# aalto-speech/AaltoASR

Measured on AMD Instinct MI355X. Metric: frames/sec GMM log-lik (39-d, 50k Gauss) + MFCC, 1/2/4/8 MI355X, higher is better.
Workload: dtype f32 (2-term fp16 split on the matrix cores, f32 accumulate); 1 GPU; configs[2]: full MFCC chain (FFT -> mel -> log -> DCT -> delta/delta-delta, CMS, normalisation) + 50000-Gaussian scoring + 2-byte LNA codes on 1 h of synthetic 16 kHz audio as 360 x 10 s utterances (449280 frames), int16 samples resident in HBM; dim=39, gaussians=50000, states=3125, gpus_flag=1

## Files before the change

### aaltoasr_amd/capi.py

```python
from __future__ import annotations

import ctypes as C
import os
import re
from typing import Optional

import numpy as np

HERE = os.path.dirname(os.path.abspath(__file__))
LIB_PATH = os.path.join(os.environ.get("AASR_LIBDIR") or os.path.join(HERE, "lib"), "libaasr.so")
HEADER_PATH = os.path.join(HERE, "..", "include", "aasr.h")

AASR_OK = 0
AASR_ERR_INVALID = -1
AASR_ERR_UNSUPPORTED = -2
AASR_ERR_NO_DEVICE = -3
AASR_ERR_IO = -4
AASR_ERR_SHORT_AUDIO = -5


class AasrError(RuntimeError):
    def __init__(self, code: int, msg: str):
        super().__init__("aasr status %d: %s" % (code, msg))
        self.code = code
# ... 596 lines not shown
        out = np.empty((n_frames, dim), dtype)
        fn = lib().aasr_feat_run if dtype == np.float32 else lib().aasr_feat_run_f64
        check(fn(self._h, _ptr(pcm), len(pcm), first_frame, n_frames,
                 module.encode() if module else None, _ptr(out)))
        return out

    def run_features(self, frames: np.ndarray, first_frame: int, n_frames: int,
                     module: Optional[str] = None, dtype=np.float32) -> np.ndarray:
        frames = np.ascontiguousarray(frames, np.float32)
        dim = self.module_dim(module) if module else self.dim
        out = np.empty((n_frames, dim), dtype)
        fn = lib().aasr_feat_run_features if dtype == np.float32 else lib().aasr_feat_run_features_f64
        check(fn(self._h, _ptr(frames), frames.size, first_frame, n_frames,
                 module.encode() if module else None, _ptr(out)))
        return out

    def run_batch_dev(self, d_pcm, pcm_off: np.ndarray, frame_off: np.ndarray, d_out, stream=None):
        pcm_off = np.ascontiguousarray(pcm_off, np.int64)
        frame_off = np.ascontiguousarray(frame_off, np.int64)
        check(lib().aasr_feat_run_batch_dev(self._h, _ptr(d_pcm), _ptr(pcm_off), _ptr(frame_off),
                                            len(pcm_off) - 1, _ptr(d_out), _stream_handle(stream)))

    def set_parameters(self, module: str, block_text: str) -> None:
        check(lib().aasr_feat_set_parameters(self._h, module.encode(), block_text.encode()))

    def get_parameters(self, module: str) -> str:
        out = C.c_void_p()
        n = C.c_int64()
        check(lib().aasr_feat_get_parameters(self._h, module.encode(), C.byref(out), C.byref(n)))
        try:
            return C.string_at(out, n.value).decode()
        finally:
            lib().aasr_free(out)

    def modules(self):
        L = lib()
        return [(L.aasr_feat_module_name(self._h, i).decode(), L.aasr_feat_module_type(self._h, i).decode())
                for i in range(L.aasr_feat_num_modules(self._h))]


def recipe_batch_range(total: int, num_batches: int, batch_index: int):
    f, n = C.c_int32(), C.c_int32()
    check(lib().aasr_recipe_batch_range(total, num_batches, batch_index, C.byref(f), C.byref(n)))
    return f.value, n.value


def debug_feat_fusion(on: bool) -> None:
    L = lib()
    L.aasr_debug_feat_fusion.argtypes = [C.c_int]
    L.aasr_debug_feat_fusion.restype = None
    L.aasr_debug_feat_fusion(int(on))


def debug_cluster_heap(on: bool) -> None:
    L = lib()
    L.aasr_debug_cluster_heap.argtypes = [C.c_int]
    L.aasr_debug_cluster_heap.restype = None
    L.aasr_debug_cluster_heap(int(on))


def recipe_frame_limits(start_time: float, end_time: float, frame_rate: float):
    a, b = C.c_int32(), C.c_int32()
    lib().aasr_recipe_frame_limits(start_time, end_time, frame_rate, C.byref(a), C.byref(b))
    return a.value, b.value


def recipe_read(text, num_batches: int = 0, batch_index: int = 0):
    out = C.c_void_p()
    n = C.c_int64()
    raw = text if isinstance(text, bytes) else text.encode()
    check(lib().aasr_recipe_read(raw, num_batches, batch_index, C.byref(out), C.byref(n)))
    try:
        table = C.string_at(out, n.value)
    finally:
        lib().aasr_free(out)
    rows = []
    for line in table.split(b"\n")[:-1]:
        f = line.split(b"\x1f")
        rows.append(tuple(x.decode("latin-1") for x in f[:4]) +
                    (float(np.float32(float(f[4]))), float(np.float32(float(f[5])))))
    return rows


def recipe_read_all(text, num_batches: int = 0, batch_index: int = 0, cluster_speakers: bool = False):
    out = C.c_void_p()
    n = C.c_int64()
    raw = text if isinstance(text, bytes) else text.encode()
    check(lib().aasr_recipe_read_all(raw, num_batches, batch_index, int(cluster_speakers), C.byref(out), C.byref(n)))
    try:
        table = C.string_at(out, n.value)
    finally:
        lib().aasr_free(out)
    rows = []
    for line in table.split(b"\n")[:-1]:
        f = [x.decode("latin-1") for x in line.split(b"\x1f")]
        rows.append(tuple(f[:7]) + (float(np.float32(float(f[7]))), float(np.float32(float(f[8]))),
                                    int(f[9]), int(f[10]), f[11], f[12]))
    return rows


def lna_read_file(path: str):
    out = C.POINTER(C.c_float)()
    S = C.c_int32()
    nb = C.c_int32()
    F = C.c_int64()
    check(lib().aasr_lna_read_file(path.encode(), C.byref(S), C.byref(nb), C.byref(F), C.byref(out)))
# ... 548 lines not shown
```

### aaltoasr_amd/csrc/feat_kernels.hip

```cpp
#include <hip/hip_runtime.h>

#include <cmath>
#include <cstring>
#include <climits>

#include "feat.h"

namespace aasr {

struct DevBatch {
  int n_utts;
  const int64_t *frame_off;
  const int64_t *pcm_off;
  const int32_t *first;
  const int32_t *eof_frame;
};

__device__ __forceinline__ int find_utt(const DevBatch &b, int64_t r, int span) {
  int lo = 0, hi = b.n_utts - 1;
  while (lo < hi) {
    int mid = (lo + hi + 1) >> 1;
    int64_t key = b.frame_off[mid] + (int64_t)mid * span;
    if (key <= r) lo = mid; else hi = mid - 1;
  }
// ... 360 lines not shown
#endif
#if AASR_ABLATION
#define AASR_FDBG(bits) (dbg & (bits))
#else
#define AASR_FDBG(bits) false
#endif
constexpr int SPEC_FRAMES = 16;
constexpr int SPEC_TPF = 16;

struct SpectralPrm {
  FftPrm fp;
  int mel_dim, mel_root, mel_terms;
  const int32_t *mel_off, *mel_t, *mel_order;
  const float *mel_scale, *mel_sum;
  int dct_dim, zeroth;
  const float *dct_cos;
};

typedef float spec_tbl_t;
struct SpectralLds {
  size_t bufs, frame_u, melv, powv, ham, perm, tw, stw, moff, mt, msc, msum, mord, dct, prm, total;
  size_t frame_u_stride;
  __host__ __device__ SpectralLds(int nc, int mel_dim, int mel_terms, int dct_rows) {
    size_t o = 0;
    auto take = [&](size_t n) {
      size_t at = o;
      o += (n + 15) & ~(size_t)15;
      return at;
    };
    bufs = take((size_t)SPEC_FRAMES * nc * 8);
    const size_t pcm_b = (size_t)(2 * nc + 2) * 2, spec_b = (size_t)((nc + 1) | 1) * 4;
    frame_u_stride = ((pcm_b > spec_b ? pcm_b : spec_b) + 7) & ~(size_t)7;
    frame_u_stride |= 4;
    frame_u = take((size_t)SPEC_FRAMES * frame_u_stride);
    melv = take((size_t)SPEC_FRAMES * mel_dim * 8);
    powv = 0;
    ham = take((size_t)2 * nc * sizeof(spec_tbl_t));
    perm = take((size_t)nc * 4);
    tw = take((size_t)nc * 8);
    stw = take((size_t)(nc / 2 + 1) * 8);
    moff = take((size_t)(mel_dim + 1) * 4);
    mt = take((size_t)mel_terms * 4);
    msc = take((size_t)mel_terms * sizeof(spec_tbl_t));
    msum = take((size_t)mel_dim * 4);
    mord = take((size_t)mel_dim * 4);
    dct = take((size_t)dct_rows * mel_dim * sizeof(spec_tbl_t));
    prm = take((size_t)SPEC_FRAMES * 3 * 8);
    total = o;
  }
};

__global__ __launch_bounds__(256) void k_spectral_fused(DevBatch b, const int16_t *__restrict__ pcm,
                                                        AudioPrm ap, int L, int R, int64_t rows,
                                                        SpectralPrm sp, int passes, int dbg,
                                                        double *__restrict__ dst) {
  extern __shared__ __attribute__((aligned(16))) char smem_raw[];
  constexpr int FB = SPEC_FRAMES, TPF = SPEC_TPF;
  const int nc = sp.fp.nc, nbins = nc + 1;
  const int dct_rows = sp.dct_dim - (sp.zeroth ? 1 : 0);
  const SpectralLds lds(nc, sp.mel_dim, sp.mel_terms, dct_rows);
  cpx *bufs = (cpx *)(smem_raw + lds.bufs);
  double *melv = (double *)(smem_raw + lds.melv);
  spec_tbl_t *t_ham = (spec_tbl_t *)(smem_raw + lds.ham);
  int32_t *t_perm = (int32_t *)(smem_raw + lds.perm);
  cpx *t_tw = (cpx *)(smem_raw + lds.tw);
  cpx *t_stw = (cpx *)(smem_raw + lds.stw);
  int32_t *t_moff = (int32_t *)(smem_raw + lds.moff);
  int32_t *t_mt = (int32_t *)(smem_raw + lds.mt);
  spec_tbl_t *t_msc = (spec_tbl_t *)(smem_raw + lds.msc);
  float *t_msum = (float *)(smem_raw + lds.msum);
  int32_t *t_mord = (int32_t *)(smem_raw + lds.mord);
  spec_tbl_t *t_dct = (spec_tbl_t *)(smem_raw + lds.dct);
  int64_t *s_prm = (int64_t *)(smem_raw + lds.prm);
  const int tid = threadIdx.x;
  const int f = tid / TPF, l = tid - f * TPF;

  for (int i = tid; i < 2 * nc; i += 256) t_ham[i] = (spec_tbl_t)sp.fp.hamming[i];
  for (int i = tid; i < nc; i += 256) {
    t_perm[i] = sp.fp.perm[i];
    t_tw[i] = ((const cpx *)sp.fp.twiddle)[i];
  }
  for (int i = tid; i < nc / 2; i += 256) t_stw[i] = ((const cpx *)sp.fp.stwiddle)[i];
  for (int i = tid; i <= sp.mel_dim; i += 256) t_moff[i] = sp.mel_off[i];
  for (int i = tid; i < sp.mel_terms; i += 256) {
    t_mt[i] = sp.mel_t[i];
    t_msc[i] = (spec_tbl_t)sp.mel_scale[i];
  }
  for (int i = tid; i < sp.mel_dim; i += 256) {
    t_msum[i] = sp.mel_sum[i];
    t_mord[i] = sp.mel_order[i];
  }
  for (int i = tid; i < dct_rows * sp.mel_dim; i += 256) t_dct[i] = (spec_tbl_t)sp.dct_cos[i];

  cpx *buf = bufs + (size_t)f * nc;
  char *fu = smem_raw + lds.frame_u + (size_t)f * lds.frame_u_stride;
  float *spec = (float *)fu;
  const int out_dim = sp.dct_dim + 1;
  const int64_t nblk = (rows + FB - 1) / FB;
  int u_cur = -1;
  for (int pass = 0; pass < passes; pass++) {
    const int64_t blk = (int64_t)blockIdx.x * passes + pass;
    if (blk >= nblk) break;
    const int64_t r0 = blk * FB;
    __syncthreads();
    if (tid < FB) {
      int64_t r = r0 + tid;
      if (r > rows - 1) r = rows - 1;
      int u;
      if (AASR_FDBG(1)) {
        u = 0;
      } else if (u_cur < 0) {
        u = find_utt_near(b, r, L + R, rows);
      } else {
        u = u_cur;
        while (u + 1 < b.n_utts && b.frame_off[u + 1] + (int64_t)(u + 1) * (L + R) <= r) u++;
      }
      u_cur = u;
      const int frame = b.first[u] - L + (int)(r - (b.frame_off[u] + (int64_t)u * (L + R)));
      s_prm[3 * tid] = window_start(b, u, frame, ap);
      s_prm[3 * tid + 1] = b.pcm_off[u];
      s_prm[3 * tid + 2] = b.pcm_off[u + 1] - b.pcm_off[u];
    }
    __syncthreads();
    {
      const int64_t ws = s_prm[3 * f], ns = s_prm[3 * f + 2];
      const int16_t *p = pcm + s_prm[3 * f + 1];
      const bool inside = ws >= 0 && ws + 2 * nc < ns;
      auto point = [&](int o) {
        const int s = t_perm[o];
        float c0, c1, c2;
        if (inside) {
          const int16_t *q = p + ws + 2 * s;
          c0 = (float)q[0];
          c1 = (float)q[1];
          c2 = (float)q[2];
        } else {
          const int64_t i = ws + 2 * s;
          c0 = (i >= 0 && i < ns) ? (float)p[i] : 0.0f;
          c1 = (i + 1 >= 0 && i + 1 < ns) ? (float)p[i + 1] : 0.0f;
          c2 = (i + 2 >= 0 && i + 2 < ns) ? (float)p[i + 2] : 0.0f;
        }
        const float p0 = ap.emph * c0, p1 = ap.emph * c1;
        cpx v;
        v.r = t_ham[2 * s] * (c1 - p0);
        v.i = t_ham[2 * s + 1] * (c2 - p1);
        return v;
      };
      for (int o = l; o < ((AASR_FDBG(32) || AASR_FDBG(8)) ? 0 : nc); o += TPF) buf[o] = point(o);
    }
    __builtin_amdgcn_fence(__ATOMIC_RELEASE, "wavefront");
    __builtin_amdgcn_wave_barrier();
    for (int st = AASR_FDBG(2) ? -1 : sp.fp.ns - 1; st >= 0; st--) {
      const int pr = sp.fp.radix[st], m = sp.fp.sublen[st];
      const int fstride = sp.fp.fstride[st];
      const int nb = fstride * m;
      for (int bi = l; bi < nb; bi += TPF) kiss_butterfly(buf, bi, pr, m, sp.fp.sub_magic[st], fstride, t_tw);
      __builtin_amdgcn_fence(__ATOMIC_RELEASE, "wavefront");
      __builtin_amdgcn_wave_barrier();
    }
    if (l == 0 && !AASR_FDBG(64)) {
      const cpx t0 = buf[0];
      spec[0] = spec_value(t0.r + t0.i, 0.0f, sp.fp.magnitude, sp.fp.take_log);
      spec[nc] = spec_value(t0.r - t0.i, 0.0f, sp.fp.magnitude, sp.fp.take_log);
    }
    for (int k0 = l; k0 < (AASR_FDBG(64) ? 0 : nc / 2); k0 += TPF) {
      const int k = k0 == 0 ? nc / 2 : k0;
      float re_k, im_k, re_n, im_n;
      real_split(buf, nc, k, t_stw, re_k, im_k, re_n, im_n);
      if (k != nc - k) spec[k] = spec_value(re_k, im_k, sp.fp.magnitude, sp.fp.take_log);
      spec[nc - k] = spec_value(re_n, im_n, sp.fp.magnitude, sp.fp.take_log);
// ... 48 lines not shown
    __builtin_amdgcn_fence(__ATOMIC_RELEASE, "wavefront");
    __builtin_amdgcn_wave_barrier();
    if (r0 + f < rows && !AASR_FDBG(128)) {
      const double *data = melv + (size_t)f * sp.mel_dim;
      for (int i = l; i < sp.dct_dim; i += TPF) {
        double acc = 0.0;
        if (sp.zeroth && i == 0) {
          for (int k = 0; k < sp.mel_dim; k++) acc += data[k];
        } else {
          const spec_tbl_t *c = t_dct + (size_t)(i - (sp.zeroth ? 1 : 0)) * sp.mel_dim;
#pragma unroll 4
          for (int k = 0; k < sp.mel_dim; k++) acc += data[k] * (double)c[k];
        }
        dst[(r0 + f) * out_dim + i] = acc;
      }
    }
    __builtin_amdgcn_fence(__ATOMIC_RELEASE, "wavefront");
    __builtin_amdgcn_wave_barrier();
  }
}

struct TemporalPrm {
  int dx, w1, w2;
  float norm1, norm2;
  const float *mean, *scale;
  const float *matrix, *bias;
  int dim;
};

#ifdef AASR_TR
constexpr int kTemporalRows = AASR_TR;
#else
constexpr int kTemporalRows = 64;
#endif

static inline size_t temporal_smem(int tile_rows, int dx, int H, int w2, int dim) {
  return (size_t)(tile_rows + 2 * H) * dx * 8 + (size_t)(tile_rows + 2 * w2) * dx * 8 + (size_t)tile_rows * 3 * dx * 8 + 16 +
         (size_t)(3 * dx) * ((dim + 2) / 3) * 16 + (size_t)(6 * dx + dim) * 4;
}

template <int ROWS, int NT>
__global__ __launch_bounds__(NT) void k_temporal_fused(DevBatch b, const double *__restrict__ src,
                                                        SrcMap sm, int span, int64_t rows,
                                                        TemporalPrm tp, int dbg, double *__restrict__ dst) {
  extern __shared__ __attribute__((aligned(16))) char smem_raw[];
  const int dx = tp.dx, H = tp.w1 + tp.w2, md = 3 * tp.dx;
  const unsigned dx_magic = fast_magic(dx), dim_magic = fast_magic(tp.dim);
  double *xs = (double *)smem_raw;
  double *d1 = xs + (size_t)(ROWS + 2 * H) * dx;
  double *nrm = d1 + (size_t)(ROWS + 2 * tp.w2) * dx;
  float4 *mt = (float4 *)(smem_raw + ((((size_t)(2 * ROWS + 2 * H + 2 * tp.w2) * dx + (size_t)ROWS * md) * 8 + 15) & ~(size_t)15));
  const int ngrp = (tp.dim + 2) / 3;
  const unsigned ngrp_magic = fast_magic(ngrp);
  if (tp.matrix && !AASR_FDBG(8))
    for (int e = threadIdx.x; e < md * ngrp; e += NT) {
      const int j = fast_div(e, ngrp_magic), g = e - j * ngrp;
      float4 v;
      v.x = tp.matrix[(size_t)(3 * g) * md + j];
      v.y = 3 * g + 1 < tp.dim ? tp.matrix[(size_t)(3 * g + 1) * md + j] : 0.0f;
      v.z = 3 * g + 2 < tp.dim ? tp.matrix[(size_t)(3 * g + 2) * md + j] : 0.0f;
      v.w = 0.0f;
      mt[e] = v;
    }
  float *nmean = (float *)(mt + (size_t)md * ngrp), *nscale = nmean + md, *nbias = nscale + md;
  for (int e = threadIdx.x; e < md; e += NT) {
    nmean[e] = tp.mean[e];
    nscale[e] = tp.scale[e];
  }
  if (tp.bias)
    for (int e = threadIdx.x; e < tp.dim; e += NT) nbias[e] = tp.bias[e];
  const int64_t tile0 = (int64_t)blockIdx.x * ROWS;
  const int64_t tile1 = tile0 + ROWS < rows ? tile0 + ROWS : rows;
  int64_t r0 = tile0;
  while (r0 < tile1) {
    const int u = AASR_FDBG(64) ? 0 : find_utt_near(b, r0, span, rows);
    const int64_t u_end = AASR_FDBG(64) ? rows : b.frame_off[u + 1] + (int64_t)(u + 1) * span;
    const int64_t r_end = u_end < tile1 ? u_end : tile1;
    const int64_t s0 = r0 + (int64_t)u * sm.span_diff + sm.shift;
    const int n_seg = (int)(r_end - r0);
    const int n_x = n_seg + 2 * H, n_d1 = n_seg + 2 * tp.w2;
    for (int e = threadIdx.x; e < (AASR_FDBG(16) ? 0 : n_x * dx); e += NT) xs[e] = src[(s0 - H) * dx + e];
    __syncthreads();
    for (int e = threadIdx.x; e < (AASR_FDBG(4) ? 0 : n_d1 * dx); e += NT) {
      const int j = fast_div(e, dx_magic), i = e - j * dx;
      const int c = j + tp.w1;
      double acc = 0;
      for (int k = 1; k <= tp.w1; k++) {
        const double left = xs[(size_t)(c - k) * dx + i];
        const double right = xs[(size_t)(c + k) * dx + i];
        acc += k * (right - left);
      }
      d1[e] = acc / (double)tp.norm1;
    }
    __syncthreads();
    for (int e = threadIdx.x; e < (AASR_FDBG(2) ? 0 : n_seg * dx); e += NT) {
      const int lr = fast_div(e, dx_magic), i = e - lr * dx;
      const double v0 = xs[(size_t)(lr + H) * dx + i];
      const double v1 = d1[(size_t)(lr + tp.w2) * dx + i];
      const int c = lr + tp.w2;
      double acc = 0;
      for (int k = 1; k <= tp.w2; k++) {
        const double left = d1[(size_t)(c - k) * dx + i];
        const double right = d1[(size_t)(c + k) * dx + i];
        acc += k * (right - left);
      }
      const double v2 = acc / (double)tp.norm2;
      double *o = nrm + (size_t)lr * md + i;
      o[0] = (v0 - (double)nmean[i]) * (double)nscale[i];
      o[dx] = (v1 - (double)nmean[dx + i]) * (double)nscale[dx + i];
      o[2 * dx] = (v2 - (double)nmean[2 * dx + i]) * (double)nscale[2 * dx + i];
    }
    __syncthreads();
    if (tp.matrix) {
      const int npair = (n_seg + 1) / 2;
      for (int it = threadIdx.x; it < ngrp * npair; it += NT) {
        const int rp = fast_div(it, ngrp_magic), g = it - rp * ngrp;
        const int la = 2 * rp, lb = 2 * rp + 1 < n_seg ? 2 * rp + 1 : la;
        const double *xa = nrm + (size_t)la * md, *xb = nrm + (size_t)lb * md;
        const float4 *mg = mt + g;
        double a0 = 0, a1 = 0, a2 = 0, b0 = 0, b1 = 0, b2 = 0;
        if (!AASR_FDBG(1)) {
#pragma unroll 3
          for (int j = 0; j < md; j++) {
            const float4 m = mg[j * ngrp];
            const double va = xa[j], vb = xb[j];
            const double m0 = (double)m.x, m1 = (double)m.y, m2 = (double)m.z;
            a0 += m0 * va;
            a1 += m1 * va;
            a2 += m2 * va;
            b0 += m0 * vb;
            b1 += m1 * vb;
            b2 += m2 * vb;
          }
        }
        const int i0 = 3 * g;
        if (tp.bias) {
          const double c0 = (double)nbias[i0];
          const double c1 = i0 + 1 < tp.dim ? (double)nbias[i0 + 1] : 0.0;
          const double c2 = i0 + 2 < tp.dim ? (double)nbias[i0 + 2] : 0.0;
          a0 += c0;
          b0 += c0;
          a1 += c1;
          b1 += c1;
          a2 += c2;
          b2 += c2;
        }
        if (AASR_FDBG(32) && a0 != 12345.0) continue;
        double *da = dst + (r0 + la) * tp.dim + i0;
        da[0] = a0;
        if (i0 + 1 < tp.dim) da[1] = a1;
        if (i0 + 2 < tp.dim) da[2] = a2;
        if (lb != la) {
          double *db = dst + (r0 + lb) * tp.dim + i0;
          db[0] = b0;
          if (i0 + 1 < tp.dim) db[1] = b1;
          if (i0 + 2 < tp.dim) db[2] = b2;
        }
      }
    } else {
      for (int e = threadIdx.x; e < n_seg * tp.dim; e += NT) {
        const int lr = fast_div(e, dim_magic), i = e - lr * tp.dim;
        double acc = nrm[(size_t)lr * md + i];
        if (tp.bias) acc += (double)nbias[i];
        dst[(r0 + lr) * tp.dim + i] = acc;
      }
    }
    __syncthreads();
    r0 = r_end;
  }
}

__global__ void k_mel(DevBatch b, const double *__restrict__ src, SrcMap sm, int span, int64_t rows,
                      int src_dim, int dim, const int32_t *__restrict__ off,
                      const int32_t *__restrict__ tt, const float *__restrict__ sc,
                      const float *__restrict__ sums, int root, double *__restrict__ dst) {
  int64_t idx = (int64_t)blockIdx.x * blockDim.x + threadIdx.x;
  if (idx >= rows * dim) return;
  int64_t r = idx / dim;
  int bin = (int)(idx - r * dim);
  const double *data = src + src_row(b, r, span, sm) * src_dim;
  float val = 0;
  for (int e = off[bin]; e < off[bin + 1]; e++)
    val = (float)((double)val + (double)sc[e] * data[tt[e]]);
  float q = (float)((double)val / (double)sums[bin]);
  double o;
  if (root) {
    o = pow((double)q, 0.1);
  } else {
    float a = q + 1.0f;
    o = (double)glibc_logf(a);
  }
  dst[idx] = o;
}

__global__ void k_power(DevBatch b, const double *__restrict__ src, SrcMap sm, int span,
                        int64_t rows, int src_dim, double *__restrict__ dst) {
  int64_t r = (int64_t)blockIdx.x * blockDim.x + threadIdx.x;
  if (r >= rows) return;
  const double *data = src + src_row(b, r, span, sm) * src_dim;
  float power = 0;
  for (int i = 0; i < src_dim; i++) power = (float)((double)power + data[i]);
  dst[r] = log((double)power + 1e-10);
}

__global__ __launch_bounds__(256) void k_power_f32src(DevBatch b, const double *__restrict__ src,
                                                      SrcMap sm, int span, int64_t rows,
                                                      int src_dim, double *__restrict__ dst) {
  const int wave = threadIdx.x >> 6, lane = threadIdx.x & 63;
  const int64_t r = (int64_t)blockIdx.x * 4 + wave;
  if (r >= rows) return;
  const double *data = src + src_row(b, r, span, sm) * src_dim;
  float power = 0;
  for (int base = 0; base < src_dim; base += 64) {
    const float v = (base + lane < src_dim) ? (float)data[base + lane] : 0.0f;
    const int cnt = src_dim - base < 64 ? src_dim - base : 64;
    if (cnt == 64) {
#pragma unroll
      for (int i = 0; i < 64; i++)
        power = power + __int_as_float(__builtin_amdgcn_readlane(__float_as_int(v), i));
    } else {
      for (int i = 0; i < cnt; i++)
// ... 231 lines not shown
  const float *w = coef + (size_t)i * stride;
  double t = 0;
  for (int j = 0, fi = start[i]; j < len[i]; j++, fi++) t += data[fi * frame_dim + d] * (double)w[j];
  const float v = (float)t;
  dst[idx] = (v < 0.0f) ? 0.0f : v;
}

__global__ void k_vtln_linear(DevBatch b, const double *__restrict__ src, SrcMap sm, int span,
                              int64_t rows, int dim, const float *__restrict__ bins,
                              double *__restrict__ dst) {
  int64_t idx = (int64_t)blockIdx.x * blockDim.x + threadIdx.x;
  if (idx >= rows * dim) return;
  int64_t r = idx / dim;
  int bi = (int)(idx - r * dim);
  const double *data = src + src_row(b, r, span, sm) * dim;
  const float pos = bins[bi];
  const float p = ceilf(pos) - pos;
  const float q = 1 - p;
  const double lo = (double)p * data[(int)floorf(pos)];
  const double hi = (double)q * data[(int)ceilf(pos)];
  dst[idx] = lo + hi;
}

__global__ void k_quanteq(DevBatch b, const double *__restrict__ src, SrcMap sm, int span,
                          int64_t rows, int dim, const float *__restrict__ alpha,
                          const float *__restrict__ gamma, const float *__restrict__ qmax,
                          double *__restrict__ dst) {
  int64_t idx = (int64_t)blockIdx.x * blockDim.x + threadIdx.x;
  if (idx >= rows * dim) return;
  int64_t r = idx / dim;
  int k = (int)(idx - r * dim);
  const double x = src[src_row(b, r, span, sm) * dim + k];
  if (!alpha) {
    dst[idx] = x;
    return;
  }
  const double ratio = x / (double)qmax[k];
  const float one_minus = 1 - alpha[k];
  const double ex = (double)gamma[k] + (double)one_minus * ratio;
  dst[idx] = (double)qmax[k] * ((double)alpha[k] * pow(ratio, ex));
}

template <class T>
__global__ void k_emit(const double *__restrict__ src, int64_t n, T *__restrict__ dst) {
  int64_t idx = (int64_t)blockIdx.x * blockDim.x + threadIdx.x;
  if (idx < n) dst[idx] = (T)src[idx];
}


static inline unsigned grid_for(int64_t n) { return (unsigned)((n + 255) / 256); }

static int g_feat_fusion = AASR_EXPERIMENT_ENV("AASR_FEAT_FUSE") ? atoi(AASR_EXPERIMENT_ENV("AASR_FEAT_FUSE")) : 1;

void feat_run_batch(aasr_feat *h, const int16_t *d_pcm, const UttBatch &ub, int target,
                    float *out_f32, double *out_f64, hipStream_t stream) {
  const int nm = (int)h->mods.size();
  const int n = ub.n_utts;
  if (n <= 0) return;
  const int64_t total = ub.frame_off[n];
  if (total <= 0) return;
  const FeatModule &base = h->mods[0];

  std::vector<int> L(nm, -1), R(nm, -1), consumers(nm, 0);
  L[target] = R[target] = 0;
  for (int i = target; i >= 0; i--) {
    if (L[i] < 0) continue;
    const FeatModule &m = h->mods[i];
    for (int s : m.sources) {
      L[s] = std::max(L[s], L[i] + m.own_left + m.lead_left);
      R[s] = std::max(R[s], R[i] + m.own_right);
      consumers[s]++;
    }
  }

  std::vector<int32_t> eof(n);
  for (int u = 0; u < n; u++) {
    int64_t ns = ub.pcm_off[u + 1] - ub.pcm_off[u];
    if (base.type == MOD_PRE) {
      if ((ub.pcm_off[u] & 1) || ns / 2 / base.dim < 1)
        raise(AASR_ERR_SHORT_AUDIO, "PreModule: Could not read the file");
      eof[u] = (int32_t)(ns / 2 / base.dim);
      continue;
    }
    if (ns < base.width + 1)
      raise(AASR_ERR_SHORT_AUDIO, "audio shorter than frame");
    if (ns > INT32_MAX)
      raise(AASR_ERR_UNSUPPORTED, "utterance longer than 2^31 samples");
    eof[u] = feat_eof_frame(h, ns);
    if (eof[u] < 1) raise(AASR_ERR_SHORT_AUDIO, "audio shorter than frame");
  }
  const size_t stage_bytes = (size_t)(n + 1) * 16 + (size_t)n * 8;
  if (h->stage_event && h->stage_busy) {
    AASR_HIP(hipEventSynchronize(h->stage_event));
    h->stage_busy = false;
  }
  if (stage_bytes > h->stage_cap) {
    if (h->stage_host) (void)hipHostFree(h->stage_host);
    h->stage_host = nullptr;
    AASR_HIP(hipHostMalloc(&h->stage_host, stage_bytes * 2, hipHostMallocDefault));
    h->stage_cap = stage_bytes * 2;
  }
  if (!h->stage_event) AASR_HIP(hipEventCreateWithFlags(&h->stage_event, hipEventDisableTiming));
  {
    char *sp = (char *)h->stage_host;
    int64_t *s_fo = (int64_t *)sp;
    int64_t *s_po = s_fo + (n + 1);
    int32_t *s_first = (int32_t *)(s_po + (n + 1));
    int32_t *s_eof = s_first + n;
    memcpy(s_fo, ub.frame_off.data(), (n + 1) * sizeof(int64_t));
// ... 49 lines not shown
      if (consumers[A] != 2 || consumers[B] != 1 || consumers[X] != 2 || A == target || B == target) continue;
      const int dx = h->mods[X].dim;
      if (h->mods[A].dim != dx || h->mods[B].dim != dx || Cm.dim != 3 * dx || T.src_dim != 3 * dx) continue;
      if ((int)h->mods[N].mean.size() != 3 * dx || (int)h->mods[N].scale.size() != 3 * dx) continue;
      const int H = h->mods[A].delta_width + h->mods[B].delta_width;
      constexpr int TR = kTemporalRows;
      if (temporal_smem(TR, dx, H, h->mods[B].delta_width, T.dim) > 64 * 1024) continue;
      tgX = X; tgA = A; tgB = B; tgN = N; tgT = ti;
      skip[A] = skip[B] = skip[C] = skip[N] = 1;
    }
  }

  auto rows_of = [&](int i) { return total + (int64_t)n * (L[i] + R[i]); };
  auto map_of = [&](int i, int s) {
    return SrcMap{(L[s] + R[s]) - (L[i] + R[i]), L[s] - L[i]};
  };

  bool emitted = false;
  for (int i = 0; i <= target; i++) {
    if (L[i] < 0 || skip[i]) continue;
    FeatModule &m = h->mods[i];
    const int64_t rows = rows_of(i);
    const int span = L[i] + R[i];
    if (i == sgG) {
      const FeatModule &F = h->mods[sgF], &M = h->mods[sgM], &D = h->mods[sgD];
      SpectralPrm sp;
      sp.fp.nc = F.fft.nc;
      sp.fp.ns = F.fft.ns;
      for (int k = 0; k < 16; k++) {
        sp.fp.radix[k] = F.fft.radix[k];
        sp.fp.sublen[k] = F.fft.sublen[k];
        sp.fp.sub_magic[k] = fast_magic(F.fft.sublen[k]);
        sp.fp.fstride[k] = k < F.fft.ns ? F.fft.nc / (F.fft.radix[k] * F.fft.sublen[k]) : 0;
      }
      sp.fp.hamming = F.fft.hamming.p;
      sp.fp.twiddle = F.fft.twiddle.p;
      sp.fp.stwiddle = F.fft.stwiddle.p;
      sp.fp.perm = F.fft.perm.p;
      sp.fp.magnitude = F.magnitude;
      sp.fp.take_log = F.take_log;
      sp.mel_dim = M.dim;
      sp.mel_root = M.root;
      sp.mel_off = M.mel_off.p;
      sp.mel_t = M.mel_t.p;
      sp.mel_scale = M.mel_scale.p;
      sp.mel_sum = M.mel_sum.p;
      sp.mel_order = M.mel_order.p;
      sp.dct_dim = D.dim;
      sp.zeroth = D.zeroth;
      sp.dct_cos = D.dct_cos.p;
      sp.mel_terms = (int)M.mel_t.n;
      const SpectralLds lds(F.fft.nc, M.dim, sp.mel_terms, D.dim - (D.zeroth ? 1 : 0));
      const int64_t nblk = (rows + SPEC_FRAMES - 1) / SPEC_FRAMES;
      const int passes = (int)std::max<int64_t>(1, std::min<int64_t>(8, nblk / 4096));
      h->bufs[i].ensure((size_t)rows * m.dim);
      hipLaunchKernelGGL(k_spectral_fused, dim3((unsigned)((nblk + passes - 1) / passes)), dim3(256), lds.total,
                         stream, db, d_pcm, ap, L[i], R[i], rows, sp, passes,
                         AASR_EXPERIMENT_ENV("AASR_SPEC_DBG") ? atoi(AASR_EXPERIMENT_ENV("AASR_SPEC_DBG")) : 0, h->bufs[i].p);
      AASR_HIP(hipGetLastError());
      continue;
    }
    if (i == tgT) {
      const FeatModule &A = h->mods[tgA], &B = h->mods[tgB], &N = h->mods[tgN];
      TemporalPrm tp;
      tp.dx = h->mods[tgX].dim;
      tp.w1 = A.delta_width;
      tp.w2 = B.delta_width;
      tp.norm1 = A.delta_norm;
      tp.norm2 = B.delta_norm;
      tp.mean = N.d_mean.p;
      tp.scale = N.d_scale.p;
      tp.matrix = m.matrix_defined ? m.d_matrix.p : nullptr;
      tp.bias = m.bias_defined ? m.d_bias.p : nullptr;
      tp.dim = m.dim;
      constexpr int TR = kTemporalRows;
      const int H = tp.w1 + tp.w2;
      const size_t smem = temporal_smem(TR, tp.dx, H, tp.w2, m.dim);
      h->bufs[i].ensure((size_t)rows * m.dim);
      constexpr int TNT = TR >= 128 ? 1024 : TR >= 64 ? 512 : 256;
      if (smem > 64 * 1024)
        AASR_HIP(hipFuncSetAttribute((const void *)k_temporal_fused<TR, TNT>, hipFuncAttributeMaxDynamicSharedMemorySize, (int)smem));
      hipLaunchKernelGGL((k_temporal_fused<TR, TNT>), dim3((unsigned)((rows + TR - 1) / TR)), dim3(TNT), smem, stream, db,
                         (const double *)h->bufs[tgX].p, map_of(i, tgX), span, rows, tp,
                         AASR_EXPERIMENT_ENV("AASR_TEMP_DBG") ? atoi(AASR_EXPERIMENT_ENV("AASR_TEMP_DBG")) : 0, h->bufs[i].p);
      AASR_HIP(hipGetLastError());
      continue;
    }
    if (m.type == MOD_AUDIOFILE && i != target && consumers[0] == 1) {
      bool only_fft = false;
      for (int j = 1; j <= target; j++)
        if (L[j] >= 0 && h->mods[j].type == MOD_FFT && h->mods[j].sources[0] == 0) only_fft = true;
      if (only_fft) continue;
    }
    h->bufs[i].ensure((size_t)rows * m.dim);
    double *dst = h->bufs[i].p;
    const int s0 = m.sources.empty() ? -1 : m.sources[0];
    const double *src = s0 >= 0 ? h->bufs[s0].p : nullptr;
    SrcMap sm = s0 >= 0 ? map_of(i, s0) : SrcMap{0, 0};
    const int64_t nelem = rows * m.dim;
    switch (m.type) {
      case MOD_PRE:
        hipLaunchKernelGGL(k_pre_frames, dim3(grid_for(nelem)), dim3(256), 0, stream, db,
                           (const float *)d_pcm, m.dim, L[i], R[i], rows, dst);
        break;
      case MOD_AUDIOFILE:
        hipLaunchKernelGGL(k_audio_frames, dim3(grid_for(nelem)), dim3(256), 0, stream, db, d_pcm,
                           ap, L[i], R[i], rows, dst);
        break;
      case MOD_FFT: {
        FftPrm fp;
        fp.nc = m.fft.nc;
        fp.ns = m.fft.ns;
        for (int k = 0; k < 16; k++) {
          fp.radix[k] = m.fft.radix[k];
          fp.sublen[k] = m.fft.sublen[k];
          fp.sub_magic[k] = fast_magic(m.fft.sublen[k]);
          fp.fstride[k] = k < m.fft.ns ? m.fft.nc / (m.fft.radix[k] * m.fft.sublen[k]) : 0;
        }
        fp.hamming = m.fft.hamming.p;
        fp.twiddle = m.fft.twiddle.p;
        fp.stwiddle = m.fft.stwiddle.p;
        fp.perm = m.fft.perm.p;
        fp.magnitude = m.magnitude;
        fp.take_log = m.take_log;
        const size_t smem = (size_t)4 * fp.nc * sizeof(float) * 2;
        const unsigned blocks = (unsigned)((rows + 3) / 4);
        bool gen = false;
        for (int st = 0; st < fp.ns; st++) gen = gen || fp.radix[st] > 5;
        const bool from_pcm = s0 == 0 && consumers[0] == 1 && target != 0;
        const double *fsrc = from_pcm ? (const double *)nullptr : src;
        if (from_pcm && gen)
          hipLaunchKernelGGL((k_fft<true, true>), dim3(blocks), dim3(256), smem, stream, db, d_pcm, ap, fsrc, sm, L[i],
                             R[i], rows, fp, dst);
        else if (from_pcm)
          hipLaunchKernelGGL((k_fft<true, false>), dim3(blocks), dim3(256), smem, stream, db, d_pcm, ap, fsrc, sm, L[i],
// ... 127 lines not shown
        AASR_HIP(hipMemcpy(dst, hout.data(), hout.size() * sizeof(double), hipMemcpyHostToDevice));
        break;
      }
      case MOD_MEAN_SUBTRACTOR: {
        const int ms_dbg = AASR_EXPERIMENT_ENV("AASR_CMS_DBG") ? atoi(AASR_EXPERIMENT_ENV("AASR_CMS_DBG")) : 0;
        auto smem_of = [&](int tile_rows) {
          const size_t n = (size_t)(tile_rows + kCmsLead + m.cms_left + m.cms_right);
          return (n + n / 8 + 1) * m.dim * 8;
        };
        int tile_rows = 0;
        if (smem_of(128) <= 78 * 1024) tile_rows = 128;
        else if (smem_of(64) <= 52 * 1024) tile_rows = 64;
        else if (smem_of(128) <= 156 * 1024) tile_rows = 128;
        else if (smem_of(64) <= 156 * 1024) tile_rows = 64;
        const bool emit_f32 = i == target && g_feat_fusion && out_f32 && !out_f64;
        auto launch = [&](auto kern, int rows_per, int nt, auto *out) {
          const size_t smem = smem_of(rows_per);
          if (smem > 64 * 1024)
            AASR_HIP(hipFuncSetAttribute((const void *)kern, hipFuncAttributeMaxDynamicSharedMemorySize, (int)smem));
          hipLaunchKernelGGL(kern, dim3((unsigned)((rows + rows_per - 1) / rows_per)), dim3(nt), smem, stream, db, src, sm,
                             span, L[i], rows, m.dim, m.cms_left, m.cms_right, ms_dbg, out);
        };
        if (tile_rows >= 128) {
          if (emit_f32) launch(k_mean_subtract_tiled<128, float, 512>, 128, 512, out_f32);
          else launch(k_mean_subtract_tiled<128, double, 512>, 128, 512, dst);
          emitted = emit_f32;
        } else if (tile_rows > 0) {
          if (emit_f32) launch(k_mean_subtract_tiled<64, float, 256>, 64, 256, out_f32);
          else launch(k_mean_subtract_tiled<64, double, 256>, 64, 256, dst);
          emitted = emit_f32;
        } else {
          hipLaunchKernelGGL(k_mean_subtract, dim3(grid_for(nelem)), dim3(256), 0, stream, db, src,
                             sm, span, rows, m.dim, m.cms_left, m.cms_right, dst);
        }
        break;
      }
    }
    AASR_HIP(hipGetLastError());
  }
  const int64_t nout = total * h->mods[target].dim;
  if (emitted) return;
  if (out_f32)
    hipLaunchKernelGGL(k_emit<float>, dim3(grid_for(nout)), dim3(256), 0, stream,
                       (const double *)h->bufs[target].p, nout, out_f32);
  if (out_f64)
    hipLaunchKernelGGL(k_emit<double>, dim3(grid_for(nout)), dim3(256), 0, stream,
                       (const double *)h->bufs[target].p, nout, out_f64);
  AASR_HIP(hipGetLastError());
}

}

extern "C" void aasr_debug_feat_fusion(int on) { aasr::g_feat_fusion = on; }
```

Baseline: 43.14 million frames/s.

## Use persistent grid-stride launches for spectral and temporal feature kernels

```diff
diff --git a/aaltoasr_amd/capi.py b/aaltoasr_amd/capi.py
--- a/aaltoasr_amd/capi.py
+++ b/aaltoasr_amd/capi.py
@@ -672,6 +672,32 @@
     L.aasr_debug_feat_fusion(int(on))
 
 
+def debug_feat_grid(workgroups: int) -> None:
+    L = lib()
+    L.aasr_debug_feat_grid.argtypes = [C.c_int]
+    L.aasr_debug_feat_grid.restype = None
+    L.aasr_debug_feat_grid(int(workgroups))
+
+
+def debug_feat_per_cu(spectral: int = 0, temporal: int = 0) -> None:
+    L = lib()
+    L.aasr_debug_feat_per_cu.argtypes = [C.c_int, C.c_int]
+    L.aasr_debug_feat_per_cu.restype = None
+    L.aasr_debug_feat_per_cu(int(spectral), int(temporal))
+
+
+def debug_feat_tile_plan(ntiles: int, cus: int, per_cu: int, cap: int = 0):
+    L = lib()
+    L.aasr_debug_feat_tile_plan.argtypes = [C.c_int64, C.c_int, C.c_int, C.c_int, C.c_void_p, C.c_void_p,
+                                            C.POINTER(C.c_int64)]
+    L.aasr_debug_feat_tile_plan.restype = C.c_int
+    room = max(1, cus) * max(1, per_cu)
+    first, count = np.zeros(room, np.int64), np.zeros(room, np.int64)
+    step = C.c_int64()
+    grid = L.aasr_debug_feat_tile_plan(ntiles, cus, per_cu, cap, _ptr(first), _ptr(count), C.byref(step))
+    return grid, first[:grid], count[:grid], step.value
+
+
 def debug_cluster_heap(on: bool) -> None:
     L = lib()
     L.aasr_debug_cluster_heap.argtypes = [C.c_int]
diff --git a/aaltoasr_amd/csrc/feat_kernels.hip b/aaltoasr_amd/csrc/feat_kernels.hip
--- a/aaltoasr_amd/csrc/feat_kernels.hip
+++ b/aaltoasr_amd/csrc/feat_kernels.hip
@@ -436,7 +436,7 @@
 
 __global__ __launch_bounds__(256) void k_spectral_fused(DevBatch b, const int16_t *__restrict__ pcm,
                                                         AudioPrm ap, int L, int R, int64_t rows,
-                                                        SpectralPrm sp, int passes, int dbg,
+                                                        SpectralPrm sp, int dbg,
                                                         double *__restrict__ dst) {
   extern __shared__ __attribute__((aligned(16))) char smem_raw[];
   constexpr int FB = SPEC_FRAMES, TPF = SPEC_TPF;
@@ -481,25 +481,14 @@
   float *spec = (float *)fu;
   const int out_dim = sp.dct_dim + 1;
   const int64_t nblk = (rows + FB - 1) / FB;
-  int u_cur = -1;
-  for (int pass = 0; pass < passes; pass++) {
-    const int64_t blk = (int64_t)blockIdx.x * passes + pass;
-    if (blk >= nblk) break;
+  int pass = 0;
+  for (int64_t blk = blockIdx.x; blk < nblk; blk += gridDim.x, pass++) {
     const int64_t r0 = blk * FB;
     __syncthreads();
     if (tid < FB) {
       int64_t r = r0 + tid;
       if (r > rows - 1) r = rows - 1;
-      int u;
-      if (AASR_FDBG(1)) {
-        u = 0;
-      } else if (u_cur < 0) {
-        u = find_utt_near(b, r, L + R, rows);
-      } else {
-        u = u_cur;
-        while (u + 1 < b.n_utts && b.frame_off[u + 1] + (int64_t)(u + 1) * (L + R) <= r) u++;
-      }
-      u_cur = u;
+      const int u = AASR_FDBG(1) ? 0 : find_utt_near(b, r, L + R, rows);
       const int frame = b.first[u] - L + (int)(r - (b.frame_off[u] + (int64_t)u * (L + R)));
       s_prm[3 * tid] = window_start(b, u, frame, ap);
       s_prm[3 * tid + 1] = b.pcm_off[u];
@@ -654,16 +643,21 @@
   float4 *mt = (float4 *)(smem_raw + ((((size_t)(2 * ROWS + 2 * H + 2 * tp.w2) * dx + (size_t)ROWS * md) * 8 + 15) & ~(size_t)15));
   const int ngrp = (tp.dim + 2) / 3;
   const unsigned ngrp_magic = fast_magic(ngrp);
-  if (tp.matrix && !AASR_FDBG(8))
+  if (tp.matrix && !AASR_FDBG(8)) {
+    const unsigned md_magic = fast_magic(md);
+    float *mtf = (float *)mt;
+    for (int e = threadIdx.x; e < tp.dim * md; e += NT) {
+      const int i = fast_div(e, md_magic), j = e - i * md;
+      const int g = i / 3;
+      mtf[((size_t)j * ngrp + g) * 4 + (i - 3 * g)] = tp.matrix[e];
+    }
     for (int e = threadIdx.x; e < md * ngrp; e += NT) {
-      const int j = fast_div(e, ngrp_magic), g = e - j * ngrp;
-      float4 v;
-      v.x = tp.matrix[(size_t)(3 * g) * md + j];
-      v.y = 3 * g + 1 < tp.dim ? tp.matrix[(size_t)(3 * g + 1) * md + j] : 0.0f;
-      v.z = 3 * g + 2 < tp.dim ? tp.matrix[(size_t)(3 * g + 2) * md + j] : 0.0f;
-      v.w = 0.0f;
-      mt[e] = v;
-    }
+      const int g = e - fast_div(e, ngrp_magic) * ngrp;
+      mtf[(size_t)e * 4 + 3] = 0.0f;
+      if (3 * g + 1 >= tp.dim) mtf[(size_t)e * 4 + 1] = 0.0f;
+      if (3 * g + 2 >= tp.dim) mtf[(size_t)e * 4 + 2] = 0.0f;
+    }
+  }
   float *nmean = (float *)(mt + (size_t)md * ngrp), *nscale = nmean + md, *nbias = nscale + md;
   for (int e = threadIdx.x; e < md; e += NT) {
     nmean[e] = tp.mean[e];
@@ -671,104 +665,105 @@
   }
   if (tp.bias)
     for (int e = threadIdx.x; e < tp.dim; e += NT) nbias[e] = tp.bias[e];
-  const int64_t tile0 = (int64_t)blockIdx.x * ROWS;
-  const int64_t tile1 = tile0 + ROWS < rows ? tile0 + ROWS : rows;
-  int64_t r0 = tile0;
-  while (r0 < tile1) {
-    const int u = AASR_FDBG(64) ? 0 : find_utt_near(b, r0, span, rows);
-    const int64_t u_end = AASR_FDBG(64) ? rows : b.frame_off[u + 1] + (int64_t)(u + 1) * span;
-    const int64_t r_end = u_end < tile1 ? u_end : tile1;
-    const int64_t s0 = r0 + (int64_t)u * sm.span_diff + sm.shift;
-    const int n_seg = (int)(r_end - r0);
-    const int n_x = n_seg + 2 * H, n_d1 = n_seg + 2 * tp.w2;
-    for (int e = threadIdx.x; e < (AASR_FDBG(16) ? 0 : n_x * dx); e += NT) xs[e] = src[(s0 - H) * dx + e];
-    __syncthreads();
-    for (int e = threadIdx.x; e < (AASR_FDBG(4) ? 0 : n_d1 * dx); e += NT) {
-      const int j = fast_div(e, dx_magic), i = e - j * dx;
-      const int c = j + tp.w1;
-      double acc = 0;
-      for (int k = 1; k <= tp.w1; k++) {
-        const double left = xs[(size_t)(c - k) * dx + i];
-        const double right = xs[(size_t)(c + k) * dx + i];
-        acc += k * (right - left);
+  for (int64_t tile0 = (int64_t)blockIdx.x * ROWS; tile0 < rows; tile0 += (int64_t)gridDim.x * ROWS) {
+    const int64_t tile1 = tile0 + ROWS < rows ? tile0 + ROWS : rows;
+    int64_t r0 = tile0;
+    while (r0 < tile1) {
+      const int u = AASR_FDBG(64) ? 0 : find_utt_near(b, r0, span, rows);
+      const int64_t u_end = AASR_FDBG(64) ? rows : b.frame_off[u + 1] + (int64_t)(u + 1) * span;
+      const int64_t r_end = u_end < tile1 ? u_end : tile1;
+      const int64_t s0 = r0 + (int64_t)u * sm.span_diff + sm.shift;
+      const int n_seg = (int)(r_end - r0);
+      const int n_x = n_seg + 2 * H, n_d1 = n_seg + 2 * tp.w2;
+      for (int e = threadIdx.x; e < (AASR_FDBG(16) ? 0 : n_x * dx); e += NT) xs[e] = src[(s0 - H) * dx + e];
+      __syncthreads();
+      for (int e = threadIdx.x; e < (AASR_FDBG(4) ? 0 : n_d1 * dx); e += NT) {
+        const int j = fast_div(e, dx_magic), i = e - j * dx;
+        const int c = j + tp.w1;
+        double acc = 0;
+        for (int k = 1; k <= tp.w1; k++) {
+          const double left = xs[(size_t)(c - k) * dx + i];
+          const double right = xs[(size_t)(c + k) * dx + i];
+          acc += k * (right - left);
+        }
+        d1[e] = acc / (double)tp.norm1;
       }
-      d1[e] = acc / (double)tp.norm1;
-    }
-    __syncthreads();
-    for (int e = threadIdx.x; e < (AASR_FDBG(2) ? 0 : n_seg * dx); e += NT) {
-      const int lr = fast_div(e, dx_magic), i = e - lr * dx;
-      const double v0 = xs[(size_t)(lr + H) * dx + i];
-      const double v1 = d1[(size_t)(lr + tp.w2) * dx + i];
-      const int c = lr + tp.w2;
-      double acc = 0;
-      for (int k = 1; k <= tp.w2; k++) {
-        const double left = d1[(size_t)(c - k) * dx + i];
-        const double right = d1[(size_t)(c + k) * dx + i];
-        acc += k * (right - left);
+      __syncthreads();
+      for (int e = threadIdx.x; e < (AASR_FDBG(2) ? 0 : n_seg * dx); e += NT) {
+        const int lr = fast_div(e, dx_magic), i = e - lr * dx;
+        const double v0 = xs[(size_t)(lr + H) * dx + i];
+        const double v1 = d1[(size_t)(lr + tp.w2) * dx + i];
+        const int c = lr + tp.w2;
+        double acc = 0;
+        for (int k = 1; k <= tp.w2; k++) {
+          const double left = d1[(size_t)(c - k) * dx + i];
+          const double right = d1[(size_t)(c + k) * dx + i];
+          acc += k * (right - left);
+        }
+        const double v2 = acc / (double)tp.norm2;
+        double *o = nrm + (size_t)lr * md + i;
+        o[0] = (v0 - (double)nmean[i]) * (double)nscale[i];
+        o[dx] = (v1 - (double)nmean[dx + i]) * (double)nscale[dx + i];
+        o[2 * dx] = (v2 - (double)nmean[2 * dx + i]) * (double)nscale[2 * dx + i];
       }
-      const double v2 = acc / (double)tp.norm2;
-      double *o = nrm + (size_t)lr * md + i;
-      o[0] = (v0 - (double)nmean[i]) * (double)nscale[i];
-      o[dx] = (v1 - (double)nmean[dx + i]) * (double)nscale[dx + i];
-      o[2 * dx] = (v2 - (double)nmean[2 * dx + i]) * (double)nscale[2 * dx + i];
-    }
-    __syncthreads();
-    if (tp.matrix) {
-      const int npair = (n_seg + 1) / 2;
-      for (int it = threadIdx.x; it < ngrp * npair; it += NT) {
-        const int rp = fast_div(it, ngrp_magic), g = it - rp * ngrp;
-        const int la = 2 * rp, lb = 2 * rp + 1 < n_seg ? 2 * rp + 1 : la;
-        const double *xa = nrm + (size_t)la * md, *xb = nrm + (size_t)lb * md;
-        const float4 *mg = mt + g;
-        double a0 = 0, a1 = 0, a2 = 0, b0 = 0, b1 = 0, b2 = 0;
-        if (!AASR_FDBG(1)) {
+      __syncthreads();
+      if (tp.matrix) {
+        const int npair = (n_seg + 1) / 2;
+        for (int it = threadIdx.x; it < ngrp * npair; it += NT) {
+          const int rp = fast_div(it, ngrp_magic), g = it - rp * ngrp;
+          const int la = 2 * rp, lb = 2 * rp + 1 < n_seg ? 2 * rp + 1 : la;
+          const double *xa = nrm + (size_t)la * md, *xb = nrm + (size_t)lb * md;
+          const float4 *mg = mt + g;
+          double a0 = 0, a1 = 0, a2 = 0, b0 = 0, b1 = 0, b2 = 0;
+          if (!AASR_FDBG(1)) {
 #pragma unroll 3
-          for (int j = 0; j < md; j++) {
-            const float4 m = mg[j * ngrp];
-            const double va = xa[j], vb = xb[j];
-            const double m0 = (double)m.x, m1 = (double)m.y, m2 = (double)m.z;
-            a0 += m0 * va;
-            a1 += m1 * va;
-            a2 += m2 * va;
-            b0 += m0 * vb;
-            b1 += m1 * vb;
-            b2 += m2 * vb;
+            for (int j = 0; j < md; j++) {
+              const float4 m = mg[j * ngrp];
+              const double va = xa[j], vb = xb[j];
+              const double m0 = (double)m.x, m1 = (double)m.y, m2 = (double)m.z;
+              a0 += m0 * va;
+              a1 += m1 * va;
+              a2 += m2 * va;
+              b0 += m0 * vb;
+              b1 += m1 * vb;
+              b2 += m2 * vb;
+            }
+          }
+          const int i0 = 3 * g;
+          if (tp.bias) {
+            const double c0 = (double)nbias[i0];
+            const double c1 = i0 + 1 < tp.dim ? (double)nbias[i0 + 1] : 0.0;
+            const double c2 = i0 + 2 < tp.dim ? (double)nbias[i0 + 2] : 0.0;
+            a0 += c0;
+            b0 += c0;
+            a1 += c1;
+            b1 += c1;
+            a2 += c2;
+            b2 += c2;
+          }
+          if (AASR_FDBG(32) && a0 != 12345.0) continue;
+          double *da = dst + (r0 + la) * tp.dim + i0;
+          da[0] = a0;
+          if (i0 + 1 < tp.dim) da[1] = a1;
+          if (i0 + 2 < tp.dim) da[2] = a2;
+          if (lb != la) {
+            double *db = dst + (r0 + lb) * tp.dim + i0;
+            db[0] = b0;
+            if (i0 + 1 < tp.dim) db[1] = b1;
+            if (i0 + 2 < tp.dim) db[2] = b2;
           }
         }
-        const int i0 = 3 * g;
-        if (tp.bias) {
-          const double c0 = (double)nbias[i0];
-          const double c1 = i0 + 1 < tp.dim ? (double)nbias[i0 + 1] : 0.0;
-          const double c2 = i0 + 2 < tp.dim ? (double)nbias[i0 + 2] : 0.0;
-          a0 += c0;
-          b0 += c0;
-          a1 += c1;
-          b1 += c1;
-          a2 += c2;
-          b2 += c2;
-        }
-        if (AASR_FDBG(32) && a0 != 12345.0) continue;
-        double *da = dst + (r0 + la) * tp.dim + i0;
-        da[0] = a0;
-        if (i0 + 1 < tp.dim) da[1] = a1;
-        if (i0 + 2 < tp.dim) da[2] = a2;
-        if (lb != la) {
-          double *db = dst + (r0 + lb) * tp.dim + i0;
-          db[0] = b0;
-          if (i0 + 1 < tp.dim) db[1] = b1;
-          if (i0 + 2 < tp.dim) db[2] = b2;
+      } else {
+        for (int e = threadIdx.x; e < n_seg * tp.dim; e += NT) {
+          const int lr = fast_div(e, dim_magic), i = e - lr * tp.dim;
+          double acc = nrm[(size_t)lr * md + i];
+          if (tp.bias) acc += (double)nbias[i];
+          dst[(r0 + lr) * tp.dim + i] = acc;
         }
       }
-    } else {
-      for (int e = threadIdx.x; e < n_seg * tp.dim; e += NT) {
-        const int lr = fast_div(e, dim_magic), i = e - lr * tp.dim;
-        double acc = nrm[(size_t)lr * md + i];
-        if (tp.bias) acc += (double)nbias[i];
-        dst[(r0 + lr) * tp.dim + i] = acc;
-      }
-    }
-    __syncthreads();
-    r0 = r_end;
+      __syncthreads();
+      r0 = r_end;
+    }
   }
 }
 
@@ -1106,9 +1101,20 @@
 
 static int g_feat_fusion = AASR_EXPERIMENT_ENV("AASR_FEAT_FUSE") ? atoi(AASR_EXPERIMENT_ENV("AASR_FEAT_FUSE")) : 1;
 
+static int g_feat_grid_cap = 0;
+static unsigned feat_persistent_grid(int64_t ntiles, int cus, int per_cu, int cap) {
+  int64_t grid = (int64_t)std::max(cus, 1) * std::max(per_cu, 1);
+  if (cap > 0) grid = std::min<int64_t>(grid, cap);
+  return (unsigned)std::max<int64_t>(1, std::min(grid, ntiles));
+}
+constexpr int kSpectralPerCu = 4, kTemporalPerCu = 3;
+static int g_spec_per_cu = kSpectralPerCu, g_temp_per_cu = kTemporalPerCu;
+
 void feat_run_batch(aasr_feat *h, const int16_t *d_pcm, const UttBatch &ub, int target,
                     float *out_f32, double *out_f64, hipStream_t stream) {
   const int nm = (int)h->mods.size();
+  int dev = 0, cus = 256;
+  if (hipGetDevice(&dev) == hipSuccess) (void)hipDeviceGetAttribute(&cus, hipDeviceAttributeMultiprocessorCount, dev);
   const int n = ub.n_utts;
   if (n <= 0) return;
   const int64_t total = ub.frame_off[n];
@@ -1264,10 +1270,9 @@
       sp.mel_terms = (int)M.mel_t.n;
       const SpectralLds lds(F.fft.nc, M.dim, sp.mel_terms, D.dim - (D.zeroth ? 1 : 0));
       const int64_t nblk = (rows + SPEC_FRAMES - 1) / SPEC_FRAMES;
-      const int passes = (int)std::max<int64_t>(1, std::min<int64_t>(8, nblk / 4096));
       h->bufs[i].ensure((size_t)rows * m.dim);
-      hipLaunchKernelGGL(k_spectral_fused, dim3((unsigned)((nblk + passes - 1) / passes)), dim3(256), lds.total,
-                         stream, db, d_pcm, ap, L[i], R[i], rows, sp, passes,
+      hipLaunchKernelGGL(k_spectral_fused, dim3(feat_persistent_grid(nblk, cus, g_spec_per_cu, g_feat_grid_cap)),
+                         dim3(256), lds.total, stream, db, d_pcm, ap, L[i], R[i], rows, sp,
                          AASR_EXPERIMENT_ENV("AASR_SPEC_DBG") ? atoi(AASR_EXPERIMENT_ENV("AASR_SPEC_DBG")) : 0, h->bufs[i].p);
       AASR_HIP(hipGetLastError());
       continue;
@@ -1292,7 +1297,8 @@
       constexpr int TNT = TR >= 128 ? 1024 : TR >= 64 ? 512 : 256;
       if (smem > 64 * 1024)
         AASR_HIP(hipFuncSetAttribute((const void *)k_temporal_fused<TR, TNT>, hipFuncAttributeMaxDynamicSharedMemorySize, (int)smem));
-      hipLaunchKernelGGL((k_temporal_fused<TR, TNT>), dim3((unsigned)((rows + TR - 1) / TR)), dim3(TNT), smem, stream, db,
+      hipLaunchKernelGGL((k_temporal_fused<TR, TNT>),
+                         dim3(feat_persistent_grid((rows + TR - 1) / TR, cus, g_temp_per_cu, g_feat_grid_cap)), dim3(TNT), smem, stream, db,
                          (const double *)h->bufs[tgX].p, map_of(i, tgX), span, rows, tp,
                          AASR_EXPERIMENT_ENV("AASR_TEMP_DBG") ? atoi(AASR_EXPERIMENT_ENV("AASR_TEMP_DBG")) : 0, h->bufs[i].p);
       AASR_HIP(hipGetLastError());
@@ -1526,3 +1532,18 @@
 }
 
 extern "C" void aasr_debug_feat_fusion(int on) { aasr::g_feat_fusion = on; }
+extern "C" void aasr_debug_feat_grid(int workgroups) { aasr::g_feat_grid_cap = workgroups; }
+extern "C" void aasr_debug_feat_per_cu(int spectral, int temporal) {
+  aasr::g_spec_per_cu = spectral > 0 ? spectral : aasr::kSpectralPerCu;
+  aasr::g_temp_per_cu = temporal > 0 ? temporal : aasr::kTemporalPerCu;
+}
+extern "C" int aasr_debug_feat_tile_plan(int64_t ntiles, int cus, int per_cu, int cap, int64_t *first, int64_t *count,
+                                         int64_t *step) {
+  const unsigned grid = aasr::feat_persistent_grid(ntiles, cus, per_cu, cap);
+  for (unsigned g = 0; g < grid; g++) {
+    first[g] = g;
+    count[g] = (int64_t)g < ntiles ? (ntiles - 1 - g) / grid + 1 : 0;
+  }
+  *step = grid;
+  return (int)grid;
+}
```

Measured after the change: 42.82 million frames/s. About the same (-0.8%).
